# lachinov/brats2019

Hardware: AMD Instinct MI355X
Metric: volumes_per_sec_fwd_bwd_128cubed_x4ch (higher is better)
Workload: dtype bf16

## Files before the change

### brats2019_amd/csrc/conv3_sb.hip

```cpp
#include "conv3_sb_common.hpp"
#include "conv3_wz_pack.hpp"
#include "conv3_mx_pack.hpp"

namespace ru {

constexpr int SB1_W_BYTES = SB_KSTEPS * 2 * 64 * 16;
template <int TZ, int TY, bool IN16, bool OUT16>
__global__ __launch_bounds__(256, 2) void conv3_sb_kernel(const Conv3Args a, const u32x4* __restrict__ wfrag, int ntz, int nty, int ntx, int nchunk) {
    using P = SB<TZ, TY>;
    constexpr int MT = P::MT, HY = P::HY, HX = P::HX, HVOLP = P::HVOLP, NSV = P::NSV, NROW = P::NROW;
    extern __shared__ __attribute__((aligned(16))) float smem[];
    u32x4* lds = reinterpret_cast<u32x4*>(smem);

    const int tid = threadIdx.x, lane = tid & 63, wave = tid >> 6;
    int b = xcd_swizzle(blockIdx.x, gridDim.x);
    const int tiles_per_sample = ntz * nty * ntx;
    const int n = b / tiles_per_sample;
    const int tis = b - n * tiles_per_sample;
    b = tis;
    const int tx = b % ntx; b /= ntx;
    const int ty = b % nty;
    const int tz = b / nty;
    const int z0 = tz * TZ, y0 = ty * TY, x0 = tx * 16;
    const int cog = blockIdx.y;
// ... 254 lines not shown
        b -= n * tiles_per_sample;
        const int tx = b % ntx; b /= ntx;
        const int ty = b % nty;
        const int tz = b / nty;
        z0 = tz * TZ; y0 = ty * TY; x0 = tx * 16;
    };

    if (producer) {
        constexpr int NPOS = NROW * HX, NR = (NPOS + 255) / 256;
        float4 va[NR], vb[NR];
        unsigned ma = 0, mb = 0;
        auto issue = [&](int item) {
            int n, z0, y0, x0;
            tile_origin(item, n, z0, y0, x0);
            const float4* xb = reinterpret_cast<const float4*>(a.x) + (size_t)n * DHW;
            ma = 0; mb = 0;
#pragma unroll
            for (int r = 0; r < NR; ++r) {
                const int p = r * 256 + ptid;
                const int row = p / HX, xc = p - row * HX;
                const int hz = row / HY, hy = row - hz * HY;
                const int gz = z0 + hz - 1, gy = y0 + hy - 1, gx = x0 + xc - 1;
                const bool rok = p < NPOS && (unsigned)gz < (unsigned)D && (unsigned)gy < (unsigned)H;
                const bool oka = rok && (unsigned)gx < (unsigned)W, okb = rok && xc + 1 < HX && (unsigned)(gx + 1) < (unsigned)W;
                const size_t rb = rok ? (size_t)(gz * H + gy) * W : 0;
                ma |= oka ? (1u << r) : 0u;
                mb |= okb ? (1u << r) : 0u;
                va[r] = xb[rb + (oka ? gx : 0)];
                vb[r] = xb[rb + (okb ? gx + 1 : 0)];
            }
        };
        auto store = [&](u32x4* buf) {
#pragma unroll
            for (int r = 0; r < NR; ++r) {
                const int p = r * 256 + ptid;
                if ((r + 1) * 256 > NPOS && p >= NPOS) continue;
                const bool oka = (ma >> r) & 1u, okb = (mb >> r) & 1u;
                const float t[8] = {oka ? va[r].x : 0.f, oka ? va[r].y : 0.f, oka ? va[r].z : 0.f, oka ? va[r].w : 0.f,
                                    okb ? vb[r].x : 0.f, okb ? vb[r].y : 0.f, okb ? vb[r].z : 0.f, okb ? vb[r].w : 0.f};
                u32x4 hi, lo;
                split8(t, hi, lo);
                buf[p] = hi;
                buf[HVOLP + p] = lo;
            }
        };
        if (nitems > 0) {
            issue(0);
            store(lds);
            if (nitems > 1) issue(1);
        }
        __syncthreads();
        for (int w = 0; w < nitems; ++w) {
            if (w + 1 < nitems) {
                store(lds + ((w + 1) & 1) * BUF);
                if (w + 2 < nitems) issue(w + 2);
            }
            __syncthreads();
        }
        __syncthreads();
    } else {
        const int mz = (rw * MT) / TY, my0 = (rw * MT) % TY;
        const int kg = lane >> 4;
        int aoff[SB4_KSTEPS];
#pragma unroll
        for (int ks = 0; ks < SB4_KSTEPS; ++ks) {
            int t = 4 * ks + kg;
            if (t > 17) t = 17;
            const int r = t >> 1, dz = r / 3, dy = r % 3, dxb = (t & 1) * 2;
            aoff[ks] = ((mz + dz) * HY + my0 + dy) * HX + dxb + (lane & 15);
        }
        u32x4 wreg[SB4_KSTEPS][2];
        {
            const u32x4* wp = wfrag + ((size_t)cog * (SB4_KSTEPS * 2)) * 64 + lane;
#pragma unroll
            for (int ks = 0; ks < SB4_KSTEPS; ++ks) {
                wreg[ks][0] = wp[(ks * 2 + 0) * 64];
                wreg[ks][1] = wp[(ks * 2 + 1) * 64];
            }
        }
        auto mm = [](const bf16x8& av, const bf16x8& wv, const f32x4& c) -> f32x4 {
            if constexpr (OUT16) return __builtin_amdgcn_mfma_f32_16x16x32_bf16(wv, av, c, 0, 0, 0);
            else return __builtin_amdgcn_mfma_f32_16x16x32_bf16(av, wv, c, 0, 0, 0);
        };
        constexpr int NS = OUT16 ? 4 : 1;
        f32x4 s1, s2;
#pragma unroll
        for (int r = 0; r < NS; ++r) { s1[r] = 0.f; s2[r] = 0.f; }
        const int stat_blk = blockIdx.x, stat_nblk = G;
        unsigned flushed = 0;
        int n_acc = -1;
        float* stat_lds = smem + BUF * 8;
        int pend_n = -1, pend_par = 0, par = 0;
        auto flush_stats = [&](int n) {
            if (a.stat_partials) sb_stats_to_lds<OUT16>(s1, s2, stat_lds + (par * 4 + rw) * 32, lane);
            pend_n = n; pend_par = par; par ^= 1;
            flushed |= 1u << (n & 31);
#pragma unroll
            for (int r = 0; r < NS; ++r) { s1[r] = 0.f; s2[r] = 0.f; }
        };
        auto commit_stats = [&]() {
            if (pend_n >= 0) {
                if (rw == 0 && a.stat_partials) sb_stats_commit(a, stat_lds + pend_par * 128, pend_n, cog, stat_blk, stat_nblk, lane);
                pend_n = -1;
            }
        };
        f32x4 acc[MT];
        __syncthreads();
        int cn, ctz, cty, ctx, gn, gz, gy, gx;
        {
            int b = swz;
            cn = b / tiles_per_sample; b -= cn * tiles_per_sample;
            ctx = b % ntx; b /= ntx;
            cty = b % nty; ctz = b / nty;
            b = G;
            gx = b % ntx; b /= ntx;
            gy = b % nty; b /= nty;
            gz = b % ntz; gn = b / ntz;
        }
        for (int w = 0; w < nitems; ++w) {
            const u32x4* buf = lds + (w & 1) * BUF;
            commit_stats();
            const int n = cn, z0 = ctz * TZ, y0 = cty * TY, x0 = ctx * 16;
            ctx += gx; if (ctx >= ntx) { ctx -= ntx; ++cty; }
            cty += gy; if (cty >= nty) { cty -= nty; ++ctz; }
            ctz += gz; if (ctz >= ntz) { ctz -= ntz; ++cn; }
            cn += gn;
            const SbOut out = sb_out_prepare<OUT16>(a, n, z0 + mz, x0, cog, lane);
            float4 radd[MT];
            const float* src = BST ? a.bst_y : a.add;
#pragma unroll
            for (int i = 0; i < MT; ++i) {
                const int yy = y0 + my0 + i;
                radd[i] = src ? *reinterpret_cast<const float4*>(src + ((out.ok && yy < H) ? sb_out_index<OUT16>(a, out, yy) : 0))
                              : make_float4(0.f, 0.f, 0.f, 0.f);
            }
            bf16x8 ah[MT], al[MT];
#pragma unroll
            for (int i = 0; i < MT; ++i) {
                ah[i] = __builtin_bit_cast(bf16x8, buf[aoff[0] + i * HX]);
                al[i] = __builtin_bit_cast(bf16x8, buf[aoff[0] + HVOLP + i * HX]);
            }
            static_for<SB4_KSTEPS>([&](auto KS) {
                constexpr int ks = decltype(KS)::value;
                constexpr bool more = ks + 1 < SB4_KSTEPS;
                const bf16x8 bh = __builtin_bit_cast(bf16x8, wreg[ks][0]);
                const bf16x8 bl = __builtin_bit_cast(bf16x8, wreg[ks][1]);
                const int nofs = aoff[more ? ks + 1 : ks];
#pragma unroll
                for (int i = 0; i < MT; ++i) {
                    if constexpr (ks == 0) acc[i] = mm(al[i], bh, f32x4{0.f, 0.f, 0.f, 0.f});
                    else acc[i] = mm(al[i], bh, acc[i]);
                    __builtin_amdgcn_sched_barrier(0);
                    if (more && i > 0) {
                        al[i - 1] = __builtin_bit_cast(bf16x8, buf[nofs + HVOLP + (i - 1) * HX]);
                        __builtin_amdgcn_sched_barrier(0);
                    }
                }
#pragma unroll
                for (int i = 0; i < MT; ++i) {
                    acc[i] = mm(ah[i], bl, acc[i]);
                    __builtin_amdgcn_sched_barrier(0);
                    if (more && i == 0) {
                        al[MT - 1] = __builtin_bit_cast(bf16x8, buf[nofs + HVOLP + (MT - 1) * HX]);
                        __builtin_amdgcn_sched_barrier(0);
                    }
                }
#pragma unroll
                for (int i = 0; i < MT; ++i) {
                    acc[i] = mm(ah[i], bh, acc[i]);
                    __builtin_amdgcn_sched_barrier(0);
                    if (more) {
                        ah[i] = __builtin_bit_cast(bf16x8, buf[nofs + i * HX]);
                        __builtin_amdgcn_sched_barrier(0);
                    }
                }
            });
            if (n != n_acc) {
                if (n_acc >= 0) flush_stats(n_acc);
                n_acc = n;
            }
            if constexpr (BST) {
                f32x4 kc[3];
                const float* kp = a.bst_k + (size_t)n * 3 * a.Cout + cog * 16 + 4 * (lane >> 4);
#pragma unroll
                for (int t = 0; t < 3; ++t) {
                    const float4 q = *reinterpret_cast<const float4*>(kp + (size_t)t * a.Cout);
                    kc[t] = f32x4{q.x, q.y, q.z, q.w};
                }
#pragma unroll
                for (int i = 0; i < MT; ++i) sb_out_tile_bst(a, out, y0 + my0 + i, acc[i], radd[i], kc, a.bst_slope, s1, s2);
            } else {
#pragma unroll
                for (int i = 0; i < MT; ++i) sb_out_tile<OUT16, NS>(a, out, y0 + my0 + i, acc[i], radd[i], s1, s2);
            }
            __syncthreads();
        }
        commit_stats();
        if (n_acc >= 0) flush_stats(n_acc);
        __syncthreads();
        commit_stats();
        if (a.stat_partials && rw == 0) {
            for (int n = 0; n < a.N; ++n)
                if (n >= 32 || !((flushed >> n) & 1u)) sb_stats_commit(a, nullptr, n, cog, stat_blk, stat_nblk, lane);
        }
    }
    fin_tail(a.fin, a.stat_partials, smem);
}

__global__ void conv3_sb_pack4_kernel(const float* __restrict__ w, u32x4* __restrict__ wfrag, int Cin_f, int Cout_f, int mode, int ncog) {
    const int i = blockIdx.x * blockDim.x + threadIdx.x;
    if (i >= ncog * SB4_KSTEPS * 64) return;
    const int lane = i & 63, ks = (i >> 6) % SB4_KSTEPS, cog = (i >> 6) / SB4_KSTEPS;
    const int col = lane & 15, g = lane >> 4, t = 4 * ks + g;
    const int cin_conv = mode == 0 ? Cin_f : Cout_f, cout_conv = mode == 0 ? Cout_f : Cin_f;
    const int co = cog * 16 + col;
    float v[8];
#pragma unroll
    for (int e = 0; e < 8; ++e) {
        const int tap = sb4_tap(t, e >> 2), ci = e & 3;
        float x = 0.f;
        if (tap >= 0 && ci < cin_conv && co < cout_conv)
            x = mode == 0 ? w[((size_t)co * Cin_f + ci) * 27 + tap] : w[((size_t)ci * Cin_f + co) * 27 + (26 - tap)];
        v[e] = x;
    }
    u32x4 hi, lo;
    split8(v, hi, lo);
    const size_t unit = ((size_t)cog * SB4_KSTEPS + ks) * 2;
    wfrag[(unit + 0) * 64 + lane] = hi;
    wfrag[(unit + 1) * 64 + lane] = lo;
}
size_t conv3_sb4_frag_bytes(int Cout_conv) { return (size_t)cdiv(Cout_conv, 16) * SB4_KSTEPS * 2 * 64 * 16; }
int conv3_sb4_pack_weights(const float* w, void* wfrag, int Cin_f, int Cout_f, int mode, hipStream_t s) {
    const int cin_conv = mode == 0 ? Cin_f : Cout_f, cout_conv = mode == 0 ? Cout_f : Cin_f;
    RU_REQUIRE(cin_conv <= 4, "conv3_sb4: at most 4 input channels");
    const int ncog = cdiv(cout_conv, 16);
    hipLaunchKernelGGL(conv3_sb_pack4_kernel, dim3(cdiv(ncog * SB4_KSTEPS * 64, 256)), dim3(256), 0, s, w, (u32x4*)wfrag, Cin_f, Cout_f, mode, ncog);
    RU_CHECK_LAUNCH("conv3_sb_pack4_kernel");
    return RU_OK;
}

__device__ __forceinline__ void sb_pack_one(const float* __restrict__ w, u32x4* __restrict__ wfrag, int Cin_f, int Cout_f, int mode, int nchunk, int ncog, int i) {
    const int total = ncog * nchunk * SB_KSTEPS * 64;
    if (i >= total) return;
    const int lane = i & 63;
    const int ks = (i >> 6) % SB_KSTEPS;
    const int chunk = ((i >> 6) / SB_KSTEPS) % nchunk;
    const int cog = (i >> 6) / (SB_KSTEPS * nchunk);
    const int col = lane & 15, g = lane >> 4;
    const int tap = sb_tap(ks, g >> 1);
    const int cin_conv = mode == 0 ? Cin_f : Cout_f, cout_conv = mode == 0 ? Cout_f : Cin_f;
    const int co = cog * 16 + col;
    float t[8];
#pragma unroll
    for (int e = 0; e < 8; ++e) {
        const int ci = chunk * 16 + (g & 1) * 8 + e;
        float v = 0.f;
        if (tap >= 0 && ci < cin_conv && co < cout_conv)
            v = mode == 0 ? w[((size_t)co * Cin_f + ci) * 27 + tap] : w[((size_t)ci * Cin_f + co) * 27 + (26 - tap)];
        t[e] = v;
    }
    u32x4 hi, lo;
    split8(t, hi, lo);
    const size_t unit = ((size_t)(cog * nchunk + chunk) * SB_KSTEPS + ks) * 2;
    wfrag[(unit + 0) * 64 + lane] = hi;
    wfrag[(unit + 1) * 64 + lane] = lo;
}
__device__ __forceinline__ void sb_pack_head_one(const float* __restrict__ w, u32x4* __restrict__ hfrag, int Cin_f, int Cout_f, int mode, int i) {
    if (i >= SB_HEAD_KSTEPS * 64) return;
    const int lane = i & 63, f = i >> 6;
    const int col = lane & 15, g = lane >> 4, dy = col >> 2, co = col & 3;
    const int tap = sb_head_tap(f, g >> 1, dy);
    const int cin_conv = mode == 0 ? Cin_f : Cout_f, cout_conv = mode == 0 ? Cout_f : Cin_f;
    float t[8];
#pragma unroll
    for (int e = 0; e < 8; ++e) {
        const int ci = (g & 1) * 8 + e;
// ... 219 lines not shown
```

### brats2019_amd/csrc/conv3_sb_common.hpp

```cpp
#pragma once
#include "conv3_epilogue.hpp"
#include "fin_tail.hpp"
#include <stdlib.h>
#include <utility>

namespace ru {


typedef __bf16 bf16x8 __attribute__((ext_vector_type(8)));
typedef unsigned int u32x4 __attribute__((ext_vector_type(4)));

constexpr int SB_KSTEPS = 14;

__host__ __device__ constexpr int sb_tap(int ks, int slot) {
    if (ks < 12) {
        const int ch = 2 * (ks / 3) + slot, dy = ks % 3;
        return (ch / 3) * 9 + dy * 3 + ch % 3;
    }
    const int dy = (ks - 12) * 2 + slot;
    return dy < 3 ? 2 * 9 + dy * 3 + 2 : -1;
}

constexpr int SB_HEAD_KSTEPS = 5;
template <int SH>
__device__ __forceinline__ float sb_row_shl(float x) {
    return __builtin_bit_cast(float, __builtin_amdgcn_update_dpp(0, __builtin_bit_cast(int, x), 0x100 + SH, 0xf, 0xf, true));
}
__host__ __device__ constexpr bool sb_head_shape(int Cin_conv, int Cout_conv) { return Cout_conv <= 4 && Cin_conv <= 16; }
__host__ __device__ constexpr int sb_head_tap(int f, int slot, int dy) {
    if (dy > 2) return -1;
    if (f < 4) return sb_tap(3 * f + dy, slot);
    return slot == 0 ? 2 * 9 + dy * 3 + 2 : -1;
}

template <int TZ, int TY>
struct SB {
    static constexpr int HZ = TZ + 2, HY = TY + 2, HX = 18;
    static constexpr int HVOL = HZ * HY * HX;
    static constexpr int HVOLP = (HVOL + 15) / 16 * 16;
    static constexpr int LDS_BYTES = 4 * HVOLP * 16;
    static constexpr int MT = TZ * TY / 4;
    static constexpr int NROW = HZ * HY;
    static constexpr int NSV = (NROW * 6 + 255) / 256;
    static_assert(MT >= 1 && TY % MT == 0, "a wave's M-tiles must lie in one z-slab");
};

typedef __bf16 bf16x2 __attribute__((ext_vector_type(2)));

__device__ __forceinline__ void split8(const float (&t)[8], u32x4& hi, u32x4& lo) {
    split_n<4>(t, hi, lo);
}

struct SbOut {
    size_t base;
    unsigned rs;
    bool ok;
    float4 bias;
};
template <bool OUT16>
__device__ __forceinline__ SbOut sb_out_prepare(const Conv3Args& a, int n, int zz, int x0, int cog, int lane) {
    SbOut o;
    const int D = a.D, H = a.H, W = a.W;
    const int zc = zz < D ? zz : 0;
    if constexpr (OUT16) {
        const int xx = x0 + (lane & 15), cq = 4 * (lane >> 4);
        o.base = ((((size_t)(n * (a.Cout >> 4) + cog) * D + zc) * H) * W + xx) * 16 + cq;
        o.rs = (unsigned)W * 16u;
        o.ok = zz < D && xx < W;
        o.bias = a.bias ? *reinterpret_cast<const float4*>(a.bias + cog * 16 + cq) : make_float4(0.f, 0.f, 0.f, 0.f);
    } else {
        const int co = cog * 16 + (lane & 15);
        const int xx = x0 + (lane >> 4) * 4;
        const int cc = co < a.Cout ? co : 0;
        o.base = (((size_t)n * a.Cout + cc) * D + zc) * (size_t)H * W + xx;
        o.rs = (unsigned)W;
        o.ok = zz < D && co < a.Cout && xx < W;
        const float b = (a.bias && co < a.Cout) ? a.bias[co] : 0.f;
        o.bias = make_float4(b, b, b, b);
    }
    return o;
}
template <bool OUT16>
__device__ __forceinline__ size_t sb_out_index(const Conv3Args& a, const SbOut& o, int yy) {
    (void)a;
    return o.base + (size_t)(unsigned)yy * o.rs;
}
template <bool OUT16, int NS>
__device__ __forceinline__ void sb_out_tile(const Conv3Args& a, const SbOut& o, int yy, f32x4 v, const float4& radd, f32x4& s1, f32x4& s2) {
    if (!(o.ok && yy < a.H)) return;
    v += f32x4{o.bias.x, o.bias.y, o.bias.z, o.bias.w} + f32x4{radd.x, radd.y, radd.z, radd.w};
    if constexpr (OUT16) {
        s1 += v;
        s2 += v * v;
    } else {
        s1[0] += (v[0] + v[1]) + (v[2] + v[3]);
        s2[0] += (v[0] * v[0] + v[1] * v[1]) + (v[2] * v[2] + v[3] * v[3]);
    }
    if constexpr (!OUT16) {
        if (a.sigmoid) {
#pragma unroll
            for (int r = 0; r < 4; ++r) v[r] = __builtin_amdgcn_rcpf(1.f + __builtin_amdgcn_exp2f(-1.44269504088896341f * v[r]));
        }
    }
    *reinterpret_cast<float4*>(a.y + sb_out_index<OUT16>(a, o, yy)) = make_float4(v[0], v[1], v[2], v[3]);
}
#ifdef RU_SB2_DBG
constexpr int kSb2RowDbg = RU_SB2_DBG;
#else
constexpr int kSb2RowDbg = 0;
#endif
template <bool OUT16, bool HAS_R, bool NT = false>
__device__ __forceinline__ void sb2_out_row(const Conv3Args& a, const SbOut& o, int yy, f32x4 v, const float4& radd, f32x4& s1, f32x4& s2) {
    if (!(o.ok && yy < a.H)) return;
    if constexpr (!OUT16) v += f32x4{o.bias.x, o.bias.y, o.bias.z, o.bias.w};
    if constexpr (HAS_R) v += f32x4{radd.x, radd.y, radd.z, radd.w};
    if constexpr (OUT16 && (kSb2RowDbg & 256)) {
        s1[0] += v[0];
    } else if constexpr (OUT16) {
        s1 += v;
        s2 += v * v;
    } else {
        s1[0] += (v[0] + v[1]) + (v[2] + v[3]);
        s2[0] += (v[0] * v[0] + v[1] * v[1]) + (v[2] * v[2] + v[3] * v[3]);
        if (a.sigmoid) {
#pragma unroll
            for (int r = 0; r < 4; ++r) v[r] = __builtin_amdgcn_rcpf(1.f + __builtin_amdgcn_exp2f(-1.44269504088896341f * v[r]));
        }
    }
    if constexpr ((kSb2RowDbg & 512) != 0) { s2[0] += v[1] + v[2] + v[3]; return; }
    if constexpr (OUT16 && NT) __builtin_nontemporal_store(v, reinterpret_cast<f32x4*>(a.y + sb_out_index<OUT16>(a, o, yy)));
    else *reinterpret_cast<float4*>(a.y + sb_out_index<OUT16>(a, o, yy)) = make_float4(v[0], v[1], v[2], v[3]);
}
template <bool NT = false>
__device__ __forceinline__ void sb_out_tile_bst(const Conv3Args& a, const SbOut& o, int yy, f32x4 v, const float4& yv, const f32x4 (&kc)[3], float slope,
                                                f32x4& s1, f32x4& s2, const float4* radd = nullptr) {
    if (!(o.ok && yy < a.H)) return;
    if (radd) v += f32x4{radd->x, radd->y, radd->z, radd->w};
    const f32x4 u = f32x4{yv.x, yv.y, yv.z, yv.w} * kc[0] + kc[1];
    const f32x4 vs = v * slope;
    f32x4 dh;
#pragma unroll
    for (int r = 0; r < 4; ++r) dh[r] = u[r] > kc[2][r] ? v[r] : vs[r];
    s1 += dh;
    s2 += dh * u;
    if constexpr (NT) __builtin_nontemporal_store(v, reinterpret_cast<f32x4*>(a.y + sb_out_index<true>(a, o, yy)));
    else *reinterpret_cast<float4*>(a.y + sb_out_index<true>(a, o, yy)) = make_float4(v[0], v[1], v[2], v[3]);
}
constexpr int SB_STAT_LDS_FLOATS = 2 * 4 * 32;
template <bool OUT16>
__device__ __forceinline__ void sb_stats_to_lds(f32x4& s1, f32x4& s2, float* sc, int lane) {
    if constexpr (OUT16) {
#pragma unroll
        for (int r = 0; r < 4; ++r) {
#pragma unroll
            for (int o = 1; o < 16; o <<= 1) { s1[r] += __shfl_xor(s1[r], o); s2[r] += __shfl_xor(s2[r], o); }
        }
        if ((lane & 15) == 0) {
#pragma unroll
            for (int r = 0; r < 4; ++r) { sc[(4 * (lane >> 4) + r) * 2] = s1[r]; sc[(4 * (lane >> 4) + r) * 2 + 1] = s2[r]; }
        }
    } else {
        s1[0] += __shfl_xor(s1[0], 16); s2[0] += __shfl_xor(s2[0], 16);
        s1[0] += __shfl_xor(s1[0], 32); s2[0] += __shfl_xor(s2[0], 32);
        if (lane < 16) { sc[lane * 2] = s1[0]; sc[lane * 2 + 1] = s2[0]; }
    }
}
__device__ __forceinline__ void sb_stats_commit(const Conv3Args& a, const float* sc4, int n, int cog, int blk, int nblk, int lane) {
    const int co = cog * 16 + lane;
    if (lane < 16 && co < a.Cout) {
        float u1 = 0.f, u2 = 0.f;
        if (sc4) {
#pragma unroll
            for (int w = 0; w < 4; ++w) { u1 += sc4[w * 32 + lane * 2]; u2 += sc4[w * 32 + lane * 2 + 1]; }
        }
        stat_publish(a.stat_partials + (((size_t)n * a.Cout + co) * nblk + blk) * 2, u1, u2);
    }
}

template <int... Is, class F>
__device__ __forceinline__ void static_for_impl(std::integer_sequence<int, Is...>, F&& f) {
    (f(std::integral_constant<int, Is>{}), ...);
}
template <int N, class F>
__device__ __forceinline__ void static_for(F&& f) {
    static_for_impl(std::make_integer_sequence<int, N>{}, static_cast<F&&>(f));
}

// ... 780 lines not shown
```

### brats2019_amd/csrc/pointwise.hip

```cpp
#include "pw_helpers.hpp"

namespace ru {

template <int VEC, int COT>
__global__ __launch_bounds__(256) void conv1_kernel(const Conv1Args a) {
    const int n = blockIdx.z;
    const int co0 = blockIdx.y * COT;
    const size_t V = a.V;
    const size_t v = ((size_t)blockIdx.x * 256 + threadIdx.x) * VEC;
    if (v >= V) return;
    float acc[COT][VEC];
#pragma unroll
    for (int o = 0; o < COT; ++o)
#pragma unroll
        for (int k = 0; k < VEC; ++k) acc[o][k] = 0.f;
    int widx[COT];
#pragma unroll
    for (int o = 0; o < COT; ++o) widx[o] = (co0 + o < a.Cout) ? co0 + o : a.Cout - 1;

    const float* xp = a.x0 + (size_t)n * a.C0 * V + v;
    const float* wr = a.wT;
#pragma unroll 4
    for (int c = 0; c < a.C0; ++c) {
        float xv[VEC];
// ... 639 lines not shown
        size_t r = i / Wh;
        const int ky = (int)(r % H); r /= H;
        const int kz = (int)(r % D);
        const size_t nc = r / D;
        const int k0 = 2 * m, k1 = 2 * m + 1;
        float wz[4], wy[4], wa[4], wb[4];
#pragma unroll
        for (int t = 0; t < 4; ++t) {
            const int oz = 2 * kz - 1 + t, oy = 2 * ky - 1 + t, oa = 2 * k0 - 1 + t, ob = 2 * k1 - 1 + t;
            wz[t] = (oz >= 0 && oz < Do) ? up2_coef(oz, D, kz) : 0.f;
            wy[t] = (oy >= 0 && oy < Ho) ? up2_coef(oy, H, ky) : 0.f;
            wa[t] = (oa >= 0 && oa < Wo) ? up2_coef(oa, W, k0) : 0.f;
            wb[t] = (ob >= 0 && ob < Wo) ? up2_coef(ob, W, k1) : 0.f;
        }
        const int oxl = 4 * m - 1 >= 0 ? 4 * m - 1 : 0, oxr = 4 * m + 4 < Wo ? 4 * m + 4 : Wo - 1;
        float acc0 = 0.f, acc1 = 0.f;
#pragma unroll
        for (int a = 0; a < 4; ++a) {
            const int oz = 2 * kz - 1 + a;
            const int ozc = oz < 0 ? 0 : (oz >= Do ? Do - 1 : oz);
            float ay0 = 0.f, ay1 = 0.f;
#pragma unroll
            for (int b = 0; b < 4; ++b) {
                const int oy = 2 * ky - 1 + b;
                const int oyc = oy < 0 ? 0 : (oy >= Ho ? Ho - 1 : oy);
                const float* p = dy + ((nc * Do + ozc) * Ho + oyc) * (size_t)Wo;
                const float4 f = *reinterpret_cast<const float4*>(p + 4 * m);
                const float fl = p[oxl], fr = p[oxr];
                ay0 += wy[b] * (wa[0] * fl + wa[1] * f.x + wa[2] * f.y + wa[3] * f.z);
                ay1 += wy[b] * (wb[0] * f.y + wb[1] * f.z + wb[2] * f.w + wb[3] * fr);
            }
            acc0 += wz[a] * ay0;
            acc1 += wz[a] * ay1;
        }
        *reinterpret_cast<float2*>(dx + ((nc * D + kz) * H + ky) * (size_t)W + 2 * m) = make_float2(acc0, acc1);
    }
}
int up2_bwd_launch(const float* dy, float* dx, int N, int C, int D, int H, int W, hipStream_t s) {
    if ((W & 1) == 0) {
        const size_t tv = (size_t)N * C * D * H * (W / 2);
        hipLaunchKernelGGL(up2_bwd_vec_kernel, dim3(grid1d(tv, 256)), dim3(256), 0, s, dy, dx, N * C, D, H, W);
        RU_CHECK_LAUNCH("up2_bwd_vec_kernel");
        return RU_OK;
    }
    const size_t total = (size_t)N * C * D * H * W;
    hipLaunchKernelGGL(up2_bwd_kernel, dim3(grid1d(total, 256)), dim3(256), 0, s, dy, dx, N * C, D, H, W);
    RU_CHECK_LAUNCH("up2_bwd_kernel");
    return RU_OK;
}

constexpr int BG_CHUNK = 16384;
size_t bias_grad_workspace_bytes(int N, int C, size_t V) { return (size_t)N * C * ((V + BG_CHUNK - 1) / BG_CHUNK) * sizeof(float); }
__global__ __launch_bounds__(256) void bias_partial_kernel(const float* __restrict__ dy, float* __restrict__ part, size_t V, int nblk) {
    __shared__ float buf[4];
    const size_t row = blockIdx.y;
    const size_t v0 = (size_t)blockIdx.x * BG_CHUNK;
    const size_t v1 = v0 + BG_CHUNK < V ? v0 + BG_CHUNK : V;
    float s1 = 0.f;
    for (size_t v = v0 + threadIdx.x; v < v1; v += 256) s1 += dy[row * V + v];
    s1 = block_sum(s1, buf);
    if (threadIdx.x == 0) part[row * nblk + blockIdx.x] = s1;
}
__global__ __launch_bounds__(256) void bias_final_kernel(const float* __restrict__ part, float* __restrict__ db, int N, int C, int nblk) {
    __shared__ double buf[4];
    const int c = blockIdx.x;
    double s1 = 0.0;
    for (int i = threadIdx.x; i < N * nblk; i += 256) {
        const int n = i / nblk, b = i % nblk;
        s1 += (double)part[((size_t)n * C + c) * nblk + b];
    }
    s1 = block_sum_d(s1, buf);
    if (threadIdx.x == 0) db[c] = (float)s1;
}
int bias_grad_launch(const float* dy, float* db, int N, int C, size_t V, void* ws, size_t ws_bytes, hipStream_t s) {
    if (!ws || ws_bytes < bias_grad_workspace_bytes(N, C, V)) { set_error("bias_grad: workspace too small"); return RU_ENOMEM; }
    const int nblk = (int)((V + BG_CHUNK - 1) / BG_CHUNK);
    hipLaunchKernelGGL(bias_partial_kernel, dim3(nblk, N * C), dim3(256), 0, s, dy, (float*)ws, V, nblk);
    RU_CHECK_LAUNCH("bias_partial_kernel");
    hipLaunchKernelGGL(bias_final_kernel, dim3(C), dim3(256), 0, s, (const float*)ws, db, N, C, nblk);
    RU_CHECK_LAUNCH("bias_final_kernel");
    return RU_OK;
}

template <bool CRIT>
__global__ __launch_bounds__(256) void head_grad_c4_kernel(const float* __restrict__ p, const float* __restrict__ dp, float* __restrict__ d4,
                                                           float* __restrict__ part, int C, size_t V, int nblk, const CritGradArgs cg) {
    __shared__ float buf[4];
    const size_t n = blockIdx.y;
    const size_t v0 = (size_t)blockIdx.x * BG_CHUNK;
    const size_t v1 = v0 + BG_CHUNK < V ? v0 + BG_CHUNK : V;
    const float* pp = p + n * C * V;
    const float* dpp = dp + n * C * V;
    float4* op = reinterpret_cast<float4*>(d4) + n * V;
    float sum[4] = {0.f, 0.f, 0.f, 0.f};
    float kg[4] = {0.f, 0.f, 0.f, 0.f}, kp[4] = {0.f, 0.f, 0.f, 0.f}, cb = 0.f;
    const float one_eps = (float)(1.0 + 1e-6);
    if constexpr (CRIT) {
        for (int c = 0; c < C && c < 4; ++c) {
            const double I = cg.sums[c] + 1e-6, U = cg.sums[C + c] + 2e-6;
            const double k = (double)cg.priority * (2.0 / (double)C) * (double)cg.w_dice;
            kg[c] = (float)(-k / U);
            kp[c] = (float)(2.0 * k * I / (U * U));
        }
        cb = (float)((double)cg.w_bce / cg.count);
    }
    for (size_t v = v0 + (size_t)threadIdx.x * 4; v < v1; v += 1024) {
        float d[4][4];
#pragma unroll
        for (int c = 0; c < 4; ++c) {
            const bool ok = c < C;
            const float4 q = *reinterpret_cast<const float4*>(pp + (ok ? c : 0) * V + v);
            float4 g = *reinterpret_cast<const float4*>(dpp + (ok ? c : 0) * V + v);
            if constexpr (CRIT) {
                const float pv[4] = {q.x, q.y, q.z, q.w}, gv[4] = {g.x, g.y, g.z, g.w};
                float o[4];
#pragma unroll
                for (int e = 0; e < 4; ++e) {
                    const float bce = -(gv[e] / (pv[e] + 1e-6f) - cg.bgw * (1.f - gv[e]) / (one_eps - pv[e]));
                    o[e] = (kg[c] * gv[e] + kp[c] * pv[e]) + cb * bce;
                }
                g = make_float4(o[0], o[1], o[2], o[3]);
            }
            d[c][0] = ok ? g.x * q.x * (1.f - q.x) : 0.f;
            d[c][1] = ok ? g.y * q.y * (1.f - q.y) : 0.f;
            d[c][2] = ok ? g.z * q.z * (1.f - q.z) : 0.f;
            d[c][3] = ok ? g.w * q.w * (1.f - q.w) : 0.f;
            sum[c] += (d[c][0] + d[c][1]) + (d[c][2] + d[c][3]);
        }
#pragma unroll
        for (int e = 0; e < 4; ++e) op[v + e] = make_float4(d[0][e], d[1][e], d[2][e], d[3][e]);
    }
#pragma unroll
    for (int c = 0; c < 4; ++c) {
        const float t = block_sum(sum[c], buf);
        if (threadIdx.x == 0 && c < C) part[(n * C + c) * nblk + blockIdx.x] = t;
    }
}
int head_grad_c4_launch(const float* p, const float* dp, float* d4, float* db, int N, int C, size_t V, void* ws, size_t ws_bytes, hipStream_t s) {
    RU_REQUIRE(C > 0 && C <= 4 && V % 4 == 0, "head_grad_c4: 1..4 channels, V % 4 == 0");
    if (!ws || ws_bytes < bias_grad_workspace_bytes(N, C, V)) { set_error("head_grad_c4: workspace too small"); return RU_ENOMEM; }
    const int nblk = (int)((V + BG_CHUNK - 1) / BG_CHUNK);
    hipLaunchKernelGGL(head_grad_c4_kernel<false>, dim3(nblk, N), dim3(256), 0, s, p, dp, d4, (float*)ws, C, V, nblk, CritGradArgs{});
    RU_CHECK_LAUNCH("head_grad_c4_kernel");
    hipLaunchKernelGGL(bias_final_kernel, dim3(C), dim3(256), 0, s, (const float*)ws, db, N, C, nblk);
    RU_CHECK_LAUNCH("bias_final_kernel");
    return RU_OK;
}
int head_grad_c4_crit_launch(const float* p, const CritGradArgs& cg, float* d4, float* db, int N, int C, size_t V, void* ws, size_t ws_bytes, hipStream_t s) {
    RU_REQUIRE(C > 0 && C <= 4 && V % 4 == 0 && cg.target && cg.sums, "head_grad_c4_crit: 1..4 channels, V % 4 == 0, target and sums");
    if (!ws || ws_bytes < bias_grad_workspace_bytes(N, C, V)) { set_error("head_grad_c4_crit: workspace too small"); return RU_ENOMEM; }
    const int nblk = (int)((V + BG_CHUNK - 1) / BG_CHUNK);
    hipLaunchKernelGGL(head_grad_c4_kernel<true>, dim3(nblk, N), dim3(256), 0, s, p, cg.target, d4, (float*)ws, C, V, nblk, cg);
    RU_CHECK_LAUNCH("head_grad_c4_kernel<crit>");
    hipLaunchKernelGGL(bias_final_kernel, dim3(C), dim3(256), 0, s, (const float*)ws, db, N, C, nblk);
    RU_CHECK_LAUNCH("bias_final_kernel");
    return RU_OK;
}

constexpr int CR_CHUNK = 8192;
int crit_tiles(size_t V) { return (int)((V + CR_CHUNK - 1) / CR_CHUNK); }
__global__ __launch_bounds__(256) void crit_partial_kernel(const float* __restrict__ p, const float* __restrict__ g, float* __restrict__ part,
                                                           size_t V, int nblk, float bgw) {
    __shared__ float buf[4];
    const size_t row = blockIdx.y;
    const size_t v0 = (size_t)blockIdx.x * CR_CHUNK;
    const size_t v1 = v0 + CR_CHUNK < V ? v0 + CR_CHUNK : V;
    const float one_eps = (float)(1.0 + 1e-6);
    float si = 0.f, su = 0.f, sb = 0.f;
    for (size_t v = v0 + threadIdx.x; v < v1; v += 256) {
        const float pv = p[row * V + v], gv = g[row * V + v];
        si += pv * gv;
        su += pv * pv + gv;
        sb += gv * logf(pv + 1e-6f) + bgw * (1.f - gv) * logf(one_eps - pv);
    }
    si = block_sum(si, buf);
    su = block_sum(su, buf);
    sb = block_sum(sb, buf);
    if (threadIdx.x == 0) {
        float* q = part + (row * nblk + blockIdx.x) * 3;
        q[0] = si; q[1] = su; q[2] = sb;
    }
}
__global__ __launch_bounds__(256) void crit_final_kernel(const float* __restrict__ part, double* __restrict__ sums, int N, int C, int nblk) {
    __shared__ double buf[4];
    double bce = 0.0;
    for (int c = 0; c < C; ++c) {
        double si = 0.0, su = 0.0, sb = 0.0;
        for (int i = threadIdx.x; i < N * nblk; i += 256) {
            const int n = i / nblk, b = i % nblk;
            const float* q = part + (((size_t)n * C + c) * nblk + b) * 3;
            si += (double)q[0]; su += (double)q[1]; sb += (double)q[2];
        }
        si = block_sum_d(si, buf);
        su = block_sum_d(su, buf);
        sb = block_sum_d(sb, buf);
        if (threadIdx.x == 0) { sums[c] = si; sums[C + c] = su; }
        bce += sb;
    }
    if (threadIdx.x == 0) sums[2 * C] = bce;
}
int crit_sums_launch(const float* p, const float* g, double* sums, int N, int C, size_t V, float bgw, void* ws, size_t ws_bytes, hipStream_t s) {
    const int nblk = crit_tiles(V);
    if (!ws || ws_bytes < (size_t)N * C * nblk * 3 * sizeof(float)) { set_error("criterion: workspace too small"); return RU_ENOMEM; }
    hipLaunchKernelGGL(crit_partial_kernel, dim3(nblk, N * C), dim3(256), 0, s, p, g, (float*)ws, V, nblk, bgw);
    RU_CHECK_LAUNCH("crit_partial_kernel");
    hipLaunchKernelGGL(crit_final_kernel, dim3(1), dim3(256), 0, s, (const float*)ws, sums, N, C, nblk);
    RU_CHECK_LAUNCH("crit_final_kernel");
    return RU_OK;
}
__global__ void crit_value_kernel(const double* __restrict__ sums, int C, double count, double priority, double w_dice, double w_bce,
                                  double* __restrict__ out) {
    double q = threadIdx.x < (unsigned)C ? 2.0 * (sums[threadIdx.x] + 1e-6) / (sums[C + threadIdx.x] + 2e-6) : 0.0;
    for (int o = 32; o > 0; o >>= 1) q += __shfl_xor(q, o);
    if (threadIdx.x == 0) {
        const double dice = priority * (1.0 - q / C), bce = -sums[2 * C] / count;
        out[0] = w_dice * dice + w_bce * bce; out[1] = dice; out[2] = bce;
    }
}
int crit_value_launch(const double* sums, int C, double count, double priority, double w_dice, double w_bce, double* out3, hipStream_t s) {
    hipLaunchKernelGGL(crit_value_kernel, dim3(1), dim3(64), 0, s, sums, C, count, priority, w_dice, w_bce, out3);
    RU_CHECK_LAUNCH("crit_value_kernel");
    return RU_OK;
}
__global__ __launch_bounds__(256) void crit_grad_kernel(const float* __restrict__ p, const float* __restrict__ g, const double* __restrict__ sums,
                                                        double count, float w_dice, float w_bce, float bgw, float priority,
                                                        float* __restrict__ dp, int C, size_t V) {
    const size_t row = blockIdx.y;
    const int c = (int)(row % C);
    const double I = sums[c] + 1e-6, U = sums[C + c] + 2e-6;
    const double k = (double)priority * (2.0 / (double)C) * (double)w_dice;
    const float cg = (float)(-k / U), cp = (float)(2.0 * k * I / (U * U));
    const float cb = (float)((double)w_bce / count);
    const float one_eps = (float)(1.0 + 1e-6);
    for (size_t v = (size_t)blockIdx.x * 256 + threadIdx.x; v < V; v += (size_t)gridDim.x * 256) {
        const float pv = p[row * V + v], gv = g[row * V + v];
// ... 351 lines not shown
```

Baseline: 274.9.

## Coalesce conv and head-grad output stores via lane shuffles and nontemporal writes

In the conv3 SB kernel, OUT16 accumulators are permuted across lanes with shuffles so each lane writes contiguous output, and the stats are shuffled back before reduction. The BST residual/row prefetch for the next work item is issued before the MFMA loop so its latency overlaps compute. Output stores use nontemporal hints. The head_grad_c4 kernel is templated on channel count, transposes its 4x4 tiles via xor shuffles for coalesced float4 stores, and also uses nontemporal stores. These add shuffle instructions and register pressure in exchange for better memory coalescing and load latency hiding.

Result: no change. 274.7 (median of 2 runs) (-0.1%).

```diff
diff --git a/brats2019_amd/csrc/conv3_sb.hip b/brats2019_amd/csrc/conv3_sb.hip
--- a/brats2019_amd/csrc/conv3_sb.hip
+++ b/brats2019_amd/csrc/conv3_sb.hip
@@ -360,6 +360,8 @@
             if constexpr (OUT16) return __builtin_amdgcn_mfma_f32_16x16x32_bf16(wv, av, c, 0, 0, 0);
             else return __builtin_amdgcn_mfma_f32_16x16x32_bf16(av, wv, c, 0, 0, 0);
         };
+        const int pl = OUT16 ? (lane >> 2) | ((lane & 3) << 4) : lane;
+        const int plinv = ((lane & 15) << 2) | (lane >> 4);
         constexpr int NS = OUT16 ? 4 : 1;
         f32x4 s1, s2;
 #pragma unroll
@@ -370,6 +372,10 @@
         float* stat_lds = smem + BUF * 8;
         int pend_n = -1, pend_par = 0, par = 0;
         auto flush_stats = [&](int n) {
+            if constexpr (OUT16) {
+#pragma unroll
+                for (int r = 0; r < NS; ++r) { s1[r] = __shfl(s1[r], plinv); s2[r] = __shfl(s2[r], plinv); }
+            }
             if (a.stat_partials) sb_stats_to_lds<OUT16>(s1, s2, stat_lds + (par * 4 + rw) * 32, lane);
             pend_n = n; pend_par = par; par ^= 1;
             flushed |= 1u << (n & 31);
@@ -383,6 +389,17 @@
             }
         };
         f32x4 acc[MT];
+        const float* src = BST ? a.bst_y : a.add;
+        auto rows_of = [&](int n, int tz, int ty, int tx, bool valid, SbOut& o, float4 (&r)[MT]) {
+            o = sb_out_prepare<OUT16>(a, n, tz * TZ + mz, tx * 16, cog, pl);
+            o.ok = o.ok && valid;
+#pragma unroll
+            for (int i = 0; i < MT; ++i) {
+                const int yy = ty * TY + my0 + i;
+                r[i] = src ? *reinterpret_cast<const float4*>(src + ((o.ok && yy < H) ? sb_out_index<OUT16>(a, o, yy) : 0))
+                           : make_float4(0.f, 0.f, 0.f, 0.f);
+            }
+        };
         __syncthreads();
         int cn, ctz, cty, ctx, gn, gz, gy, gx;
         {
@@ -395,23 +412,21 @@
             gy = b % nty; b /= nty;
             gz = b % ntz; gn = b / ntz;
         }
+        SbOut out;
+        float4 radd[MT];
+        if constexpr (BST) rows_of(cn, ctz, cty, ctx, nitems > 0, out, radd);
         for (int w = 0; w < nitems; ++w) {
             const u32x4* buf = lds + (w & 1) * BUF;
             commit_stats();
-            const int n = cn, z0 = ctz * TZ, y0 = cty * TY, x0 = ctx * 16;
+            const int n = cn, y0 = cty * TY;
+            if constexpr (!BST) rows_of(cn, ctz, cty, ctx, true, out, radd);
             ctx += gx; if (ctx >= ntx) { ctx -= ntx; ++cty; }
             cty += gy; if (cty >= nty) { cty -= nty; ++ctz; }
             ctz += gz; if (ctz >= ntz) { ctz -= ntz; ++cn; }
             cn += gn;
-            const SbOut out = sb_out_prepare<OUT16>(a, n, z0 + mz, x0, cog, lane);
-            float4 radd[MT];
-            const float* src = BST ? a.bst_y : a.add;
-#pragma unroll
-            for (int i = 0; i < MT; ++i) {
-                const int yy = y0 + my0 + i;
-                radd[i] = src ? *reinterpret_cast<const float4*>(src + ((out.ok && yy < H) ? sb_out_index<OUT16>(a, out, yy) : 0))
-                              : make_float4(0.f, 0.f, 0.f, 0.f);
-            }
+            SbOut onext;
+            float4 rnext[BST ? MT : 1];
+            if constexpr (BST) rows_of(cn, ctz, cty, ctx, w + 1 < nitems, onext, rnext);
             bf16x8 ah[MT], al[MT];
 #pragma unroll
             for (int i = 0; i < MT; ++i) {
@@ -457,19 +472,29 @@
                 if (n_acc >= 0) flush_stats(n_acc);
                 n_acc = n;
             }
+            if constexpr (OUT16) {
+#pragma unroll
+                for (int i = 0; i < MT; ++i) {
+#pragma unroll
+                    for (int r = 0; r < 4; ++r) acc[i][r] = __shfl(acc[i][r], pl);
+                }
+            }
             if constexpr (BST) {
                 f32x4 kc[3];
-                const float* kp = a.bst_k + (size_t)n * 3 * a.Cout + cog * 16 + 4 * (lane >> 4);
+                const float* kp = a.bst_k + (size_t)n * 3 * a.Cout + cog * 16 + 4 * (pl >> 4);
 #pragma unroll
                 for (int t = 0; t < 3; ++t) {
                     const float4 q = *reinterpret_cast<const float4*>(kp + (size_t)t * a.Cout);
                     kc[t] = f32x4{q.x, q.y, q.z, q.w};
                 }
 #pragma unroll
-                for (int i = 0; i < MT; ++i) sb_out_tile_bst(a, out, y0 + my0 + i, acc[i], radd[i], kc, a.bst_slope, s1, s2);
+                for (int i = 0; i < MT; ++i) sb_out_tile_bst<true>(a, out, y0 + my0 + i, acc[i], radd[i], kc, a.bst_slope, s1, s2);
+                out = onext;
+#pragma unroll
+                for (int i = 0; i < MT; ++i) radd[i] = rnext[i];
             } else {
 #pragma unroll
-                for (int i = 0; i < MT; ++i) sb_out_tile<OUT16, NS>(a, out, y0 + my0 + i, acc[i], radd[i], s1, s2);
+                for (int i = 0; i < MT; ++i) sb_out_tile<OUT16, NS, OUT16>(a, out, y0 + my0 + i, acc[i], radd[i], s1, s2);
             }
             __syncthreads();
         }
diff --git a/brats2019_amd/csrc/conv3_sb_common.hpp b/brats2019_amd/csrc/conv3_sb_common.hpp
--- a/brats2019_amd/csrc/conv3_sb_common.hpp
+++ b/brats2019_amd/csrc/conv3_sb_common.hpp
@@ -85,7 +85,7 @@
     (void)a;
     return o.base + (size_t)(unsigned)yy * o.rs;
 }
-template <bool OUT16, int NS>
+template <bool OUT16, int NS, bool NT = false>
 __device__ __forceinline__ void sb_out_tile(const Conv3Args& a, const SbOut& o, int yy, f32x4 v, const float4& radd, f32x4& s1, f32x4& s2) {
     if (!(o.ok && yy < a.H)) return;
     v += f32x4{o.bias.x, o.bias.y, o.bias.z, o.bias.w} + f32x4{radd.x, radd.y, radd.z, radd.w};
@@ -102,7 +102,8 @@
             for (int r = 0; r < 4; ++r) v[r] = __builtin_amdgcn_rcpf(1.f + __builtin_amdgcn_exp2f(-1.44269504088896341f * v[r]));
         }
     }
-    *reinterpret_cast<float4*>(a.y + sb_out_index<OUT16>(a, o, yy)) = make_float4(v[0], v[1], v[2], v[3]);
+    if constexpr (NT) __builtin_nontemporal_store(v, reinterpret_cast<f32x4*>(a.y + sb_out_index<OUT16>(a, o, yy)));
+    else *reinterpret_cast<float4*>(a.y + sb_out_index<OUT16>(a, o, yy)) = make_float4(v[0], v[1], v[2], v[3]);
 }
 #ifdef RU_SB2_DBG
 constexpr int kSb2RowDbg = RU_SB2_DBG;
diff --git a/brats2019_amd/csrc/pointwise.hip b/brats2019_amd/csrc/pointwise.hip
--- a/brats2019_amd/csrc/pointwise.hip
+++ b/brats2019_amd/csrc/pointwise.hip
@@ -745,7 +745,7 @@
     return RU_OK;
 }
 
-template <bool CRIT>
+template <bool CRIT, int NC>
 __global__ __launch_bounds__(256) void head_grad_c4_kernel(const float* __restrict__ p, const float* __restrict__ dp, float* __restrict__ d4,
                                                            float* __restrict__ part, int C, size_t V, int nblk, const CritGradArgs cg) {
     __shared__ float buf[4];
@@ -754,7 +754,7 @@
     const size_t v1 = v0 + BG_CHUNK < V ? v0 + BG_CHUNK : V;
     const float* pp = p + n * C * V;
     const float* dpp = dp + n * C * V;
-    float4* op = reinterpret_cast<float4*>(d4) + n * V;
+    f32x4_pw* op = reinterpret_cast<f32x4_pw*>(d4) + n * V;
     float sum[4] = {0.f, 0.f, 0.f, 0.f};
     float kg[4] = {0.f, 0.f, 0.f, 0.f}, kp[4] = {0.f, 0.f, 0.f, 0.f}, cb = 0.f;
     const float one_eps = (float)(1.0 + 1e-6);
@@ -767,15 +767,23 @@
         }
         cb = (float)((double)cg.w_bce / cg.count);
     }
-    for (size_t v = v0 + (size_t)threadIdx.x * 4; v < v1; v += 1024) {
-        float d[4][4];
-#pragma unroll
-        for (int c = 0; c < 4; ++c) {
+    const int q = threadIdx.x & 3;
+    const size_t qb = v0 + (size_t)(threadIdx.x >> 2) * 16;
+#pragma unroll 4
+    for (int k = 0; k < BG_CHUNK / 1024; ++k) {
+        const size_t v = v0 + (size_t)threadIdx.x * 4 + (size_t)k * 1024;
+        const bool act = v < v1;
+        const size_t vl = act ? v : v0;
+        f32x4_pw t[4];
+#pragma unroll
+        for (int e = 0; e < 4; ++e) t[e] = f32x4_pw{0.f, 0.f, 0.f, 0.f};
+#pragma unroll
+        for (int c = 0; c < NC; ++c) {
             const bool ok = c < C;
-            const float4 q = *reinterpret_cast<const float4*>(pp + (ok ? c : 0) * V + v);
-            float4 g = *reinterpret_cast<const float4*>(dpp + (ok ? c : 0) * V + v);
+            const float4 qv = *reinterpret_cast<const float4*>(pp + (ok ? c : 0) * V + vl);
+            float4 g = *reinterpret_cast<const float4*>(dpp + (ok ? c : 0) * V + vl);
             if constexpr (CRIT) {
-                const float pv[4] = {q.x, q.y, q.z, q.w}, gv[4] = {g.x, g.y, g.z, g.w};
+                const float pv[4] = {qv.x, qv.y, qv.z, qv.w}, gv[4] = {g.x, g.y, g.z, g.w};
                 float o[4];
 #pragma unroll
                 for (int e = 0; e < 4; ++e) {
@@ -784,26 +792,46 @@
                 }
                 g = make_float4(o[0], o[1], o[2], o[3]);
             }
-            d[c][0] = ok ? g.x * q.x * (1.f - q.x) : 0.f;
-            d[c][1] = ok ? g.y * q.y * (1.f - q.y) : 0.f;
-            d[c][2] = ok ? g.z * q.z * (1.f - q.z) : 0.f;
-            d[c][3] = ok ? g.w * q.w * (1.f - q.w) : 0.f;
-            sum[c] += (d[c][0] + d[c][1]) + (d[c][2] + d[c][3]);
-        }
-#pragma unroll
-        for (int e = 0; e < 4; ++e) op[v + e] = make_float4(d[0][e], d[1][e], d[2][e], d[3][e]);
+            const float d0 = ok ? g.x * qv.x * (1.f - qv.x) : 0.f;
+            const float d1 = ok ? g.y * qv.y * (1.f - qv.y) : 0.f;
+            const float d2 = ok ? g.z * qv.z * (1.f - qv.z) : 0.f;
+            const float d3 = ok ? g.w * qv.w * (1.f - qv.w) : 0.f;
+            if (act) sum[c] += (d0 + d1) + (d2 + d3);
+            t[0][c] = d0; t[1][c] = d1; t[2][c] = d2; t[3][c] = d3;
+        }
+#pragma unroll
+        for (int st = 1; st <= 2; st <<= 1) {
+            const bool up = (q & st) != 0;
+#pragma unroll
+            for (int e = 0; e < 4; ++e) {
+                if (e & st) continue;
+                f32x4_pw give = up ? t[e] : t[e + st], got;
+#pragma unroll
+                for (int r = 0; r < 4; ++r) got[r] = __shfl_xor(give[r], st);
+                if (up) t[e] = got; else t[e + st] = got;
+            }
+        }
+        const size_t w0 = qb + (size_t)k * 1024 + q;
+#pragma unroll
+        for (int i = 0; i < 4; ++i)
+            if (w0 + 4 * i < v1) __builtin_nontemporal_store(t[i], op + w0 + 4 * i);
     }
 #pragma unroll
     for (int c = 0; c < 4; ++c) {
         const float t = block_sum(sum[c], buf);
         if (threadIdx.x == 0 && c < C) part[(n * C + c) * nblk + blockIdx.x] = t;
     }
+}
+template <bool CRIT>
+static void head_grad_c4_run(const float* p, const float* dp, float* d4, float* ws, int N, int C, size_t V, int nblk, const CritGradArgs& cg, hipStream_t s) {
+    if (C == 3) hipLaunchKernelGGL((head_grad_c4_kernel<CRIT, 3>), dim3(nblk, N), dim3(256), 0, s, p, dp, d4, ws, C, V, nblk, cg);
+    else hipLaunchKernelGGL((head_grad_c4_kernel<CRIT, 4>), dim3(nblk, N), dim3(256), 0, s, p, dp, d4, ws, C, V, nblk, cg);
 }
 int head_grad_c4_launch(const float* p, const float* dp, float* d4, float* db, int N, int C, size_t V, void* ws, size_t ws_bytes, hipStream_t s) {
     RU_REQUIRE(C > 0 && C <= 4 && V % 4 == 0, "head_grad_c4: 1..4 channels, V % 4 == 0");
     if (!ws || ws_bytes < bias_grad_workspace_bytes(N, C, V)) { set_error("head_grad_c4: workspace too small"); return RU_ENOMEM; }
     const int nblk = (int)((V + BG_CHUNK - 1) / BG_CHUNK);
-    hipLaunchKernelGGL(head_grad_c4_kernel<false>, dim3(nblk, N), dim3(256), 0, s, p, dp, d4, (float*)ws, C, V, nblk, CritGradArgs{});
+    head_grad_c4_run<false>(p, dp, d4, (float*)ws, N, C, V, nblk, CritGradArgs{}, s);
     RU_CHECK_LAUNCH("head_grad_c4_kernel");
     hipLaunchKernelGGL(bias_final_kernel, dim3(C), dim3(256), 0, s, (const float*)ws, db, N, C, nblk);
     RU_CHECK_LAUNCH("bias_final_kernel");
@@ -813,7 +841,7 @@
     RU_REQUIRE(C > 0 && C <= 4 && V % 4 == 0 && cg.target && cg.sums, "head_grad_c4_crit: 1..4 channels, V % 4 == 0, target and sums");
     if (!ws || ws_bytes < bias_grad_workspace_bytes(N, C, V)) { set_error("head_grad_c4_crit: workspace too small"); return RU_ENOMEM; }
     const int nblk = (int)((V + BG_CHUNK - 1) / BG_CHUNK);
-    hipLaunchKernelGGL(head_grad_c4_kernel<true>, dim3(nblk, N), dim3(256), 0, s, p, cg.target, d4, (float*)ws, C, V, nblk, cg);
+    head_grad_c4_run<true>(p, cg.target, d4, (float*)ws, N, C, V, nblk, cg, s);
     RU_CHECK_LAUNCH("head_grad_c4_kernel<crit>");
     hipLaunchKernelGGL(bias_final_kernel, dim3(C), dim3(256), 0, s, (const float*)ws, db, N, C, nblk);
     RU_CHECK_LAUNCH("bias_final_kernel");
```
